# epruesse/SINA

Measured on AMD Instinct MI355X. Metric: aligned sequences/sec (whole node), 100k full-length 16S vs SILVA-NR-scale ref, higher is better.
Workload: dtype f32

## Files before the change

sina_amd/csrc/graph_build.hip:

```cpp
#include <algorithm>
#include <cstring>
#include <type_traits>

#include "common.h"
#include "ctx.h"

namespace sina_hip {
namespace {

#ifndef SINA_GRAPH_THREADS
#define SINA_GRAPH_THREADS 512
#endif
#ifndef SINA_GRAPH_MINWAVES
#define SINA_GRAPH_MINWAVES 8
#endif
constexpr int kGT = SINA_GRAPH_THREADS;
constexpr uint32_t kNoPrev = 0xFFFFu;
constexpr int kMaxFam = kFamilyMax;
#ifndef SINA_GRAPH_KTC
#define SINA_GRAPH_KTC 128
#endif
#ifndef SINA_GRAPH_TNW
#define SINA_GRAPH_TNW 512
#endif
constexpr int kTC = SINA_GRAPH_KTC;
constexpr int kTNW = SINA_GRAPH_TNW;
static_assert(kTC % 64 == 0 && kTC < 255 && kTNW >= 32 && kTNW % 2 == 0, "tile geometry");
static_assert((kMaxFam * (kTC / 64) + SINA_GRAPH_THREADS / 64 - 1) / (SINA_GRAPH_THREADS / 64) <= 64, "far-entry flags of a wave fit 64 bits");

#ifdef SINA_DP_PROFILE
__device__ unsigned long long g_graph_prof[16];
#define GP_DECL unsigned long long gp_[16] = {}; unsigned long long gt_ = __builtin_amdgcn_s_memtime();
#define GP(i) { const unsigned long long t_ = __builtin_amdgcn_s_memtime(); gp_[i] += t_ - gt_; gt_ = t_; }
#define GP_FLUSH if (threadIdx.x == 0) { for (int i_ = 0; i_ < 16; i_++) atomicAdd(&g_graph_prof[i_], gp_[i_]); }
#else
#define GP_DECL
#define GP(i)
#define GP_FLUSH
#endif

struct GraphArgs {
    const uint32_t *ref_ab;
    const uint64_t *ref_off;
    const uint32_t *fam_ids;
    const uint64_t *fam_off;
    const uint64_t *pred_off;
    const float *wtab;
    uint4 *rec;
    uint32_t *node_pos;
    uint32_t *succ_min;
    uint32_t *far_mark;
    uint32_t *pred;
    uint2 *pred4;
    uint32_t *sizes;
    uint16_t *chain_rows;
    uint32_t width, ncap;
    uint32_t tile_bytes;
    uint32_t bitmap_off;
    uint32_t member_off;
    uint32_t member_cap;
    uint32_t fam_cap;
    int W;
    int want_smin;
    uint2 *reach;
    float kappa64;
};

struct Member {
    uint64_t beg;
    uint32_t len;
    uint32_t cur, curn;
    uint32_t carry, carryn;
    uint32_t id;
};
static_assert(sizeof(Member) == 32, "LDS layout");
constexpr uint32_t kOCpos = 0;
constexpr uint32_t kONbase = kOCpos + 4 * kTC;
constexpr uint32_t kOPres = kONbase + 4 * (kTC + 2);
constexpr uint32_t kOWA = kOPres + 4 * kTC;
constexpr uint32_t kOWC = kOWA + 4 * kTNW;
constexpr uint32_t kOWD = kOWC + 4 * kTNW;
constexpr uint32_t kOWB = (kOWD + 4 * kTNW + 7) & ~7u;
constexpr uint32_t kOLi = kOWB + 8 * kTNW;
constexpr uint32_t kONn = kOLi + 32 * kTC;
constexpr uint32_t kONfar = kONn + kTC;
constexpr uint32_t kOMask = kONfar + kTNW;
constexpr uint32_t kONcol = kOMask + kTNW;
constexpr uint32_t kOE = (kONcol + kTNW + 15) & ~15u;
constexpr int kELower0Bit = 14;
constexpr uint32_t kODot16 = kTC + 1;

template <typename In, typename Out>
__device__ uint32_t block_exscan(const In *in, Out *out, uint32_t n, uint32_t *tmp) {
    const uint32_t tid = threadIdx.x;
    const uint32_t chunk = (n + kGT - 1) / kGT;
    const uint32_t b = min(n, tid * chunk), e = min(n, b + chunk);
    uint32_t s = 0;
    for (uint32_t i = b; i < e; i++) s += (uint32_t)in[i];
    uint32_t x = s;
    const int lane = tid & 63, wave = tid >> 6;
#pragma unroll
    for (int off = 1; off < 64; off <<= 1) {
        const uint32_t y = __shfl_up(x, off);
        if (lane >= off) x += y;
    }
    if (lane == 63) tmp[wave] = x;
    __syncthreads();
    uint32_t base = 0, total = 0;
    for (int w = 0; w < kGT / 64; w++) {
        if (w < wave) base += tmp[w];
        total += tmp[w];
    }
    uint32_t run = base + x - s;
    __syncthreads();
    for (uint32_t i = b; i < e; i++) {
        const uint32_t v = (uint32_t)in[i];
        out[i] = (Out)run;
        run += v;
    }
    __syncthreads();
    return total;
}

template <typename Get, typename Out>
__device__ uint32_t block_exscan_f(uint32_t n, Get get, Out *out, uint32_t *tmp) {
    const uint32_t tid = threadIdx.x;
    const uint32_t chunk = (n + kGT - 1) / kGT;
    const uint32_t b = min(n, tid * chunk), e = min(n, b + chunk);
    uint32_t s = 0;
    for (uint32_t i = b; i < e; i++) s += get(i);
    uint32_t x = s;
    const int lane = tid & 63, wave = tid >> 6;
#pragma unroll
    for (int off = 1; off < 64; off <<= 1) {
        const uint32_t y = __shfl_up(x, off);
        if (lane >= off) x += y;
    }
    if (lane == 63) tmp[wave] = x;
    __syncthreads();
    uint32_t base = 0, total = 0;
    for (int w = 0; w < kGT / 64; w++) {
        if (w < wave) base += tmp[w];
        total += tmp[w];
    }
    uint32_t run = base + x - s;
    __syncthreads();
    for (uint32_t i = b; i < e; i++) {
        const uint32_t v = get(i);
        out[i] = (Out)run;
        run += v;
    }
    __syncthreads();
    return total;
}

__device__ uint32_t block_incscan(uint32_t *v, uint32_t n, uint32_t *tmp) {
    const uint32_t tid = threadIdx.x;
    const uint32_t chunk = (n + kGT - 1) / kGT;
    const uint32_t b = min(n, tid * chunk), e = min(n, b + chunk);
    uint32_t s = 0;
    for (uint32_t i = b; i < e; i++) s += v[i];
    uint32_t x = s;
    const int lane = tid & 63, wave = tid >> 6;
#pragma unroll
    for (int off = 1; off < 64; off <<= 1) {
        const uint32_t y = __shfl_up(x, off);
        if (lane >= off) x += y;
    }
    if (lane == 63) tmp[wave] = x;
    __syncthreads();
    uint32_t base = 0, total = 0;
    for (int w = 0; w < kGT / 64; w++) {
        if (w < wave) base += tmp[w];
        total += tmp[w];
    }
    uint32_t run = base + x - s;
    for (uint32_t i = b; i < e; i++) {
        run += v[i];
        v[i] = run;
    }
    __syncthreads();
    return total;
}

constexpr uint32_t kCdSpilled = 1u << 16, kCdNone = 1u << 17, kCdSink = 1u << 30, kCdFence = 1u << 31;
__device__ __forceinline__ uint32_t row_of_code(uint32_t c) {
    return (c & kCdNone) ? kRowNone : (c & kCdSpilled) ? (kRowSpilled | (c & 0xFFFFu)) : (c & 0xFFFFu);
}

template <int K, typename Get, typename Put>
__device__ __forceinline__ uint32_t slot_walk(uint32_t b, uint32_t e, int W, Get get, Put put) {
    uint32_t fa[K];
#pragma unroll
    for (int x = 0; x < K; x++) fa[x] = (x < W) ? 0u : 0xFFFFFFFFu;
    uint32_t nsp = 0;
    for (uint32_t m = b; m < e; m++) {
        const uint32_t cd = get(m);
        const uint32_t l = cd & 0xFFFFu;
        uint32_t c = kCdNone;
        if (!(cd & kCdSink) && l != m + 1) {
            const bool may_slot = !(cd & kCdFence) && l < e;
            uint32_t slot = K;
#pragma unroll
            for (int x = K - 1; x >= 0; x--) slot = (may_slot && fa[x] <= m) ? (uint32_t)x : slot;
#pragma unroll
            for (int x = 0; x < K; x++) fa[x] = (slot == (uint32_t)x) ? l : fa[x];
            c = slot < (uint32_t)K ? slot : (kCdSpilled | nsp++);
        }
        put(m, cd, c);
    }
    return nsp;
}

__device__ __attribute__((noinline)) void fill_tile(const uint32_t *__restrict__ ref_ab, uint32_t bitmap_off, uint32_t member_off,
                                                    uint32_t nwords, uint32_t n_tasks, uint32_t c0, uint32_t tc) {
    extern __shared__ __attribute__((aligned(16))) unsigned char smem[];
    uint32_t *cposT = reinterpret_cast<uint32_t *>(smem + kOCpos);
    uint32_t *presT = reinterpret_cast<uint32_t *>(smem + kOPres);
    uint16_t *eE = reinterpret_cast<uint16_t *>(smem + kOE);
    const uint32_t *bitmap = reinterpret_cast<const uint32_t *>(smem + bitmap_off);
    const uint16_t *wrank = reinterpret_cast<const uint16_t *>(bitmap + nwords);
    Member *mb = reinterpret_cast<Member *>(smem + member_off);
    constexpr uint32_t kEAbsent = 0x00FFu, kEFirst = 1u << 13;
    constexpr uint32_t kCH = kTC / 64, kNW = kGT / 64;
    const uint32_t wave = (uint32_t)__builtin_amdgcn_readfirstlane((int)(threadIdx.x >> 6));
    const uint32_t lane = threadIdx.x & 63u;
    auto rank = [&](uint32_t pos) -> uint32_t {
        return (uint32_t)wrank[pos >> 5] + __popc(bitmap[pos >> 5] & ((1u << (pos & 31)) - 1u));
    };
        for (uint32_t t4 = wave; t4 < n_tasks; t4 += 8 * kNW) {
            uint32_t abv[8];
#pragma unroll
            for (int u = 0; u < 8; u++) {
                const uint32_t task = t4 + (uint32_t)u * kNW;
                abv[u] = 0xFFFFFFFFu;
                if (task < n_tasks) {
                    const uint32_t j = task / kCH;
                    const uint32_t cur = (uint32_t)__builtin_amdgcn_readfirstlane((int)mb[j].cur);
                    const uint32_t len = (uint32_t)__builtin_amdgcn_readfirstlane((int)mb[j].len);
                    const uint64_t beg = mb[j].beg;
                    const uint64_t begs = ((uint64_t)(uint32_t)__builtin_amdgcn_readfirstlane((int)(uint32_t)(beg >> 32)) << 32) |
                                          (uint32_t)__builtin_amdgcn_readfirstlane((int)(uint32_t)beg);
                    const uint32_t i = cur + (task % kCH) * 64u + lane;
                    if (i < len) abv[u] = ref_ab[begs + i];
                }
            }
#pragma unroll
            for (int u = 0; u < 8; u++) {
                const uint32_t task = t4 + (uint32_t)u * kNW;
                if (task >= n_tasks) continue;
                const uint32_t j = task / kCH, slot0 = (task % kCH) * 64u, slot = slot0 + lane;
                const uint32_t cur = (uint32_t)__builtin_amdgcn_readfirstlane((int)mb[j].cur);
                uint32_t ev = kEAbsent;
                if (abv[u] != 0xFFFFFFFFu) {
                    const uint32_t ab = abv[u];
                    const uint32_t pos = ab & 0xFFFFFFu;
                    const uint32_t c = rank(pos) - c0;
                    if (c < tc) {
                        const uint32_t m = (ab >> 24) & 0x1Fu;
                        ev = c | (m << 8) | (cur + slot == 0 ? kEFirst : 0u);
                        atomicOr(&presT[c], 1u << m);
                        cposT[c] = pos;
                    }
                }
                eE[j * (uint32_t)kTC + slot] = (uint16_t)ev;
                const uint32_t n_in = (uint32_t)__popcll(__builtin_amdgcn_ballot_w64(ev != kEAbsent));
                if (n_in && lane == 0) atomicMax(&mb[j].curn, cur + slot0 + n_in);
            }
        }
}

__device__ __forceinline__ uint32_t node_of_entry(uint32_t ev) {
    extern __shared__ __attribute__((aligned(16))) unsigned char smem[];
    const uint32_t *nbaseT = reinterpret_cast<const uint32_t *>(smem + kONbase);
    const uint32_t *presT = reinterpret_cast<const uint32_t *>(smem + kOPres);
    const uint8_t *liOf = smem + kOLi;
    const uint32_t c = ev & 0xFFu, m = (ev >> 8) & 31u;
    const uint32_t b = nbaseT[c];
    return b + liOf[b + __popc(presT[c] & ((1u << m) - 1u))];
}
__device__ __attribute__((noinline)) void merge_dot16(uint32_t n_tasks) {
    extern __shared__ __attribute__((aligned(16))) unsigned char smem[];
    const uint32_t *presT = reinterpret_cast<const uint32_t *>(smem + kOPres);
    uint16_t *eE = reinterpret_cast<uint16_t *>(smem + kOE);
    for (uint32_t e = threadIdx.x; e < n_tasks * 64u; e += kGT) {
        const uint32_t ev = eE[e];
        const uint32_t c = ev & 0xFFu;
        if (c != 0xFFu && ((ev >> 8) & 31u) == 16u && !(presT[c] & 0x10000u)) eE[e] = (uint16_t)((ev & ~(31u << 8)) | (1u << kELower0Bit));
    }
}
__device__ __attribute__((noinline)) void fix_dot16(uint32_t n_tasks, uint32_t ca, uint32_t cb, uint32_t w0) {
    extern __shared__ __attribute__((aligned(16))) unsigned char smem[];
    const uint32_t *nbaseT = reinterpret_cast<const uint32_t *>(smem + kONbase);
    const uint32_t *wC = reinterpret_cast<const uint32_t *>(smem + kOWC);
    const uint16_t *eE = reinterpret_cast<const uint16_t *>(smem + kOE);
    uint8_t *maskN = smem + kOMask;
    for (uint32_t e = threadIdx.x; e < n_tasks * 64u; e += kGT) {
        const uint32_t ev = eE[e];
        const uint32_t c = ev & 0xFFu;
        if (c >= ca && c < cb && (ev >> kELower0Bit) && wC[nbaseT[c] - w0] == e / (uint32_t)kTC) maskN[node_of_entry(ev) - w0] = 16;
    }
}
__global__ void __launch_bounds__(kGT) __attribute__((amdgpu_waves_per_eu(SINA_GRAPH_MINWAVES, SINA_GRAPH_MINWAVES))) family_graph_kernel(GraphArgs a) {
    extern __shared__ __attribute__((aligned(16))) unsigned char smem[];
    __shared__ uint32_t s_tmp[kGT / 64 + 8];
    const uint32_t q = blockIdx.x, tid = threadIdx.x;
    const uint32_t nwords = (a.width + 31) / 32;
    const uint64_t f0 = a.fam_off[q];
    const uint32_t F = (uint32_t)(a.fam_off[q + 1] - f0);
    uint32_t *cposT = reinterpret_cast<uint32_t *>(smem + kOCpos);
    uint32_t *nbaseT = reinterpret_cast<uint32_t *>(smem + kONbase);
    uint32_t *presT = reinterpret_cast<uint32_t *>(smem + kOPres);
    uint32_t *wA = reinterpret_cast<uint32_t *>(smem + kOWA);
    uint32_t *wC = reinterpret_cast<uint32_t *>(smem + kOWC);
    uint32_t *wD = reinterpret_cast<uint32_t *>(smem + kOWD);
    unsigned long long *wB = reinterpret_cast<unsigned long long *>(smem + kOWB);
    uint8_t *liOf = smem + kOLi;
    uint8_t *nn = smem + kONn;
    uint8_t *nfarN = smem + kONfar;
    uint8_t *maskN = smem + kOMask;
    uint8_t *ncolN = smem + kONcol;
    uint16_t *eE = reinterpret_cast<uint16_t *>(smem + kOE);
    uint32_t *bitmap = reinterpret_cast<uint32_t *>(smem + a.bitmap_off);
    uint16_t *wrank = reinterpret_cast<uint16_t *>(bitmap + nwords);
    Member *mb = reinterpret_cast<Member *>(smem + a.member_off);
    constexpr uint32_t kEFirst = 1u << 13;
    constexpr uint32_t kCH = kTC / 64, kNW = kGT / 64;
    const uint32_t wave = (uint32_t)__builtin_amdgcn_readfirstlane((int)(threadIdx.x >> 6));
    const uint32_t lane = threadIdx.x & 63u;
    const uint32_t n_tasks = F * kCH;

    uint32_t *sz = a.sizes + kBuiltWords * (size_t)q;
    for (uint32_t j = tid; j < F; j += kGT) {
        const uint32_t id = a.fam_ids[f0 + j];
        mb[j].id = id;
        mb[j].beg = a.ref_off[id];
        mb[j].len = (uint32_t)(a.ref_off[id + 1] - a.ref_off[id]);
        mb[j].cur = mb[j].curn = 0;
        mb[j].carry = mb[j].carryn = kNoPrev;
    }
    for (uint32_t i = tid; i < nwords; i += kGT) bitmap[i] = 0;
    if (tid == 0) nbaseT[kODot16] = 0;
    __syncthreads();
    GP_DECL

    for (uint32_t j0 = 0; j0 < F; j0 += 8) {
        uint32_t maxlen = 0;
#pragma unroll
        for (int u = 0; u < 8; u++) maxlen = max(maxlen, j0 + u < F ? mb[j0 + u].len : 0u);
        for (uint32_t i = tid; i < maxlen; i += kGT) {
            uint32_t ab[8];
#pragma unroll
            for (int u = 0; u < 8; u++)
                ab[u] = (j0 + u < F && i < mb[j0 + u].len) ? a.ref_ab[mb[j0 + u].beg + i] : 0xFFFFFFFFu;
#pragma unroll
            for (int u = 0; u < 8; u++)
                if (ab[u] != 0xFFFFFFFFu) {
                    const uint32_t pos = ab[u] & 0xFFFFFFu;
                    atomicOr(&bitmap[pos >> 5], 1u << (pos & 31));
                }
        }
    }
    __syncthreads();
    GP(0)
    {
        const uint32_t chunk = (nwords + kGT - 1) / kGT;
        const uint32_t b = min(nwords, tid * chunk), e = min(nwords, b + chunk);
        uint32_t s = 0;
        for (uint32_t i = b; i < e; i++) s += __popc(bitmap[i]);
        uint32_t x = s;
        const int lane = tid & 63, wave = tid >> 6;
#pragma unroll
        for (int off = 1; off < 64; off <<= 1) {
            const uint32_t y = __shfl_up(x, off);
            if (lane >= off) x += y;
        }
        if (lane == 63) s_tmp[wave] = x;
        __syncthreads();
        uint32_t base = 0, total = 0;
        for (int w = 0; w < kGT / 64; w++) {
            if (w < wave) base += s_tmp[w];
            total += s_tmp[w];
        }
        uint32_t run = base + x - s;
        for (uint32_t i = b; i < e; i++) {
            wrank[i] = (uint16_t)run;
            run += __popc(bitmap[i]);
        }
        if (tid == 0) s_tmp[kGT / 64] = total;
    }
    __syncthreads();
    const uint32_t NC = s_tmp[kGT / 64];
    if (NC > 65535u) {
        if (tid == 0) {
            sz[kBuiltN] = NC;
            sz[kBuiltEdges] = sz[kBuiltSpill] = 0;
            sz[kBuiltStatus] = kBuiltNodeCap;
        }
        return;
    }
    auto rank = [&](uint32_t pos) -> uint32_t {
        return (uint32_t)wrank[pos >> 5] + __popc(bitmap[pos >> 5] & ((1u << (pos & 31)) - 1u));
    };
    uint4 *rec = a.rec + (size_t)q * a.ncap;
    uint32_t *node_pos = a.node_pos + (size_t)q * a.ncap;
    uint32_t *smin = a.succ_min + (size_t)q * a.ncap;
    uint32_t *last = a.far_mark + (size_t)q * a.ncap;
    uint32_t *pred = a.pred + a.pred_off[q];
    uint16_t *chain_rows = a.chain_rows + (size_t)q * a.ncap;
    const float *wt = a.wtab + (size_t)F * (kMaxFam + 1);
    uint32_t N = 0, E = 0;
    GP(1)

    for (uint32_t c0 = 0; c0 < NC; c0 += kTC) {
        const uint32_t tc = min((uint32_t)kTC, NC - c0);
        for (uint32_t i = tid; i < (uint32_t)kTC; i += kGT) presT[i] = 0;
        __syncthreads();
        GP(2)
        fill_tile(a.ref_ab, a.bitmap_off, a.member_off, nwords, n_tasks, c0, tc);
        __syncthreads();
        for (uint32_t c = tid; c < tc; c += kGT) {
            uint32_t p = presT[c];
            if ((p & 0x10001u) == 0x10001u) {
                p &= ~0x10000u;
                presT[c] = p;
                nbaseT[kODot16] = 1u;
            }
            nn[c] = (uint8_t)__popc(p);
        }
        __syncthreads();
        if (nbaseT[kODot16]) {
            merge_dot16(n_tasks);
            __syncthreads();
        }
        GP(3)
        const uint32_t tn = block_exscan(nn, nbaseT, tc, s_tmp);
        if (tid == 0) nbaseT[tc] = tn;
        for (uint32_t ln = tid; ln < tn; ln += kGT)
            if (N + ln < a.ncap) {
                last[N + ln] = 0;
                if (a.want_smin) smin[N + ln] = 0xFFFFFFFFu;
            }
        __syncthreads();
        GP(5)
        uint32_t te = 0;
        for (uint32_t ca = 0; ca < tc;) {
            const uint32_t w0 = nbaseT[ca];
            uint32_t cb = tc;
            if (tn - w0 > (uint32_t)kTNW) {
                uint32_t lo = ca + 1, hi = tc;
                while (lo < hi) {
                    const uint32_t mid = (lo + hi + 1) / 2;
                    if (nbaseT[mid] - w0 <= (uint32_t)kTNW) lo = mid;
                    else hi = mid - 1;
                }
                cb = lo;
            }
            const uint32_t wn = nbaseT[cb] - w0;
            for (uint32_t i = tid; i < wn; i += kGT) {
                wA[i] = 0;
                wB[i] = 0;
                wC[i] = 0xFFFFFFFFu;
                nfarN[i] = 0;
            }
            __syncthreads();
            for (uint32_t task = wave; task < n_tasks; task += kNW) {
                const uint32_t j = task / kCH, slot = (task % kCH) * 64u + lane;
                const uint32_t ev = eE[j * (uint32_t)kTC + slot];
                const uint32_t c = ev & 0xFFu;
                if (c >= ca && c < cb) {
                    const uint32_t m = (ev >> 8) & 31u;
                    atomicMin(&wC[nbaseT[c] + __popc(presT[c] & ((1u << m) - 1u)) - w0], j);
                }
            }
            __syncthreads();
            for (uint32_t c = ca + tid; c < cb; c += kGT) {
                const uint32_t base = nbaseT[c], k = nn[c];
                uint32_t pp = presT[c];
                for (uint32_t x = 0; x < k; x++) {
                    const uint32_t mj = wC[base - w0 + x];
                    uint32_t r = 0;
                    for (uint32_t y = 0; y < k; y++) r += (wC[base - w0 + y] < mj) ? 1u : 0u;
                    liOf[base + x] = (uint8_t)r;
                    maskN[base - w0 + r] = (uint8_t)(__ffs(pp) - 1);
                    ncolN[base - w0 + r] = (uint8_t)c;
                    pp &= pp - 1u;
                }
            }
            __syncthreads();
            if (nbaseT[kODot16]) {
                fix_dot16(n_tasks, ca, cb, w0);
                __syncthreads();
            }
            GP(4)
            auto node_of = [&](uint32_t ev) -> uint32_t { return node_of_entry(ev); };
            unsigned long long farbits = 0;
            {
                uint32_t it = 0;
                for (uint32_t task = wave; task < n_tasks; task += kNW, it++) {
                    const uint32_t j = task / kCH, slot = (task % kCH) * 64u + lane;
                    const uint32_t ev = eE[j * (uint32_t)kTC + slot];
                    const uint32_t c = ev & 0xFFu;
                    const bool mine = c >= ca && c < cb;
                    const uint32_t ln = mine ? node_of(ev) : 0u;
                    uint32_t lnp = __shfl_up(ln, 1);
                    const bool left_mine = __shfl_up(mine ? 1 : 0, 1) != 0;
                    if (!mine) continue;
                    const uint32_t node = N + ln;
                    const bool first = (ev & kEFirst) != 0;
                    atomicAdd(&wA[ln - w0], first ? 1u : 0x10001u);
                    if (mb[j].cur + slot + 1 == mb[j].curn) mb[j].carryn = node;
                    if (j == 0 && mb[0].cur + slot < a.ncap) chain_rows[mb[0].cur + slot] = (uint16_t)node;
                    if (!first) {
                        if (slot && (lane == 0 || !left_mine)) lnp = node_of(eE[j * (uint32_t)kTC + slot - 1]);
                        const uint32_t pn = slot ? N + lnp : mb[j].carry;
                        const uint32_t d = node - pn;
                        if (d <= 64u) atomicOr(&wB[ln - w0], 1ull << (d - 1u));
                        else farbits |= 1ull << it;
                    }
                }
            }
            for (uint32_t i = tid; i < wn; i += kGT) wC[i] = 0xFFFFFFFFu;
            __syncthreads();
            GP(6)
            const uint32_t te_w = block_exscan_f(wn, [&](uint32_t i) { return wA[i] >> 16; }, wD, s_tmp);
            while (__syncthreads_or(farbits != 0 ? 1 : 0)) {
                uint32_t it = 0;
                for (uint32_t task = wave; task < n_tasks; task += kNW, it++) {
                    if (!((farbits >> it) & 1ull)) continue;
                    const uint32_t j = task / kCH, slot = (task % kCH) * 64u + lane;
                    const uint32_t ln = node_of(eE[j * (uint32_t)kTC + slot]);
                    const uint32_t pn = slot ? N + node_of(eE[j * (uint32_t)kTC + slot - 1]) : mb[j].carry;
                    atomicMin(&wC[ln - w0], pn);
                }
                __syncthreads();
                it = 0;
                for (uint32_t task = wave; task < n_tasks; task += kNW, it++) {
                    if (!((farbits >> it) & 1ull)) continue;
                    const uint32_t j = task / kCH, slot = (task % kCH) * 64u + lane;
                    const uint32_t ln = node_of(eE[j * (uint32_t)kTC + slot]);
                    const uint32_t pn = slot ? N + node_of(eE[j * (uint32_t)kTC + slot - 1]) : mb[j].carry;
                    if (wC[ln - w0] == pn) farbits &= ~(1ull << it);
                }
                __syncthreads();
                for (uint32_t i = tid; i < wn; i += kGT) {
                    const uint32_t v = wC[i];
                    if (v == 0xFFFFFFFFu) continue;
                    const uint32_t node = N + w0 + i;
                    if (node < a.ncap) {
                        pred[E + te + wD[i] + nfarN[i]] = v;
                        if (a.want_smin) atomicMin(&smin[v], cposT[ncolN[i]]);
                        atomicMax(&last[v], node);
                    }
                    nfarN[i]++;
                    wC[i] = 0xFFFFFFFFu;
                }
            }
            for (uint32_t i = tid; i < wn; i += kGT) {
                const uint32_t node = N + w0 + i;
                if (node >= a.ncap) continue;
                const uint32_t seg = E + te + wD[i];
                const uint32_t pos = cposT[ncolN[i]];
                uint32_t np = nfarN[i];
                unsigned long long bits = wB[i];
                while (bits) {
                    const uint32_t hi = 63u - (uint32_t)__clzll((long long)bits);
                    bits ^= 1ull << hi;
                    const uint32_t pa = node - (hi + 1u);
                    pred[seg + np] = pa;
                    np++;
                    if (a.want_smin) atomicMin(&smin[pa], pos);
                    atomicMax(&last[pa], node);
                }
                uint4 r;
                r.x = seg;
                r.y = __float_as_uint(wt[wA[i] & 0xFFFFu]);
                r.z = (np & 0xFFu) | ((uint32_t)maskN[i] << 8);
                r.w = kRowNone;
                rec[node] = r;
                node_pos[node] = pos;
            }
            te += te_w;
            ca = cb;
            __syncthreads();
        }
        for (uint32_t j = tid; j < F; j += kGT) {
            mb[j].cur = mb[j].curn;
            mb[j].carry = mb[j].carryn;
        }
        N += tn;
        E += te;
        __syncthreads();
        GP(7)
    }
    if (N > a.ncap || N > 65535u) {
        if (tid == 0) {
            sz[kBuiltN] = N;
            sz[kBuiltEdges] = sz[kBuiltSpill] = 0;
            sz[kBuiltStatus] = kBuiltNodeCap;
        }
        return;
    }
    GP(8)
    const uint32_t seg_len = dp_slot_segment(N);
    const uint32_t n_seg = (N + seg_len - 1) / seg_len;
    uint32_t *codeL = reinterpret_cast<uint32_t *>(smem);
    const bool in_lds = (size_t)N * 4 <= a.tile_bytes;
    const bool beside = a.reach != nullptr && (size_t)N * 8 <= a.tile_bytes;
    uint32_t *cwL = codeL + N;
    constexpr int kSFirstSink = kGT / 64 + 1, kSGmin = kGT / 64 + 2, kSSpill = kGT / 64 + 3;
    if (tid == 0) {
        s_tmp[kSFirstSink] = 0xFFFFFFFFu;
        s_tmp[kSGmin] = 0xFFFFFFFFu;
    }
    __syncthreads();
    for (uint32_t i = tid; i < N; i += kGT) {
        const uint32_t l = last[i];
        uint32_t cd = l;
        if (l == 0) {
            cd |= kCdSink;
            atomicMin(&s_tmp[kSFirstSink], i);
            if (a.want_smin) smin[i] = 1000000u;
        }
        if (l > i && l - i > (uint32_t)kFarLds) cd |= kCdFence;
        if (in_lds) codeL[i] = cd;
        else if (cd & (kCdSink | kCdFence)) rec[i].z |= ((cd & kCdSink) ? kRecSink : 0u) | ((cd & kCdFence) ? kRecFence : 0u);
    }
    auto column_maxima = [&](uint32_t *cw, uint32_t first, uint32_t step) {
        for (uint32_t i = first; i < N; i += step) {
            const uint32_t pos = node_pos[i];
            if (i > 0 && node_pos[i - 1] == pos) continue;
            uint32_t mx = 0;
            for (uint32_t j = i; j < N && node_pos[j] == pos; j++) {
                mx = max(mx, prune_gain_units(__uint_as_float(rec[j].y), a.kappa64));
                cw[j] = 0;
            }
            cw[i] = mx;
            atomicMin(&s_tmp[kSGmin], mx);
        }
    };
    __syncthreads();
    GP(9)
    if (wave == 0) {
        uint32_t nsp = 0;
        if (tid < n_seg) {
            const uint32_t b = tid * seg_len, e = min(N, b + seg_len);
            auto walk = [&](auto kslots) {
                constexpr int K = decltype(kslots)::value;
                if (in_lds)
                    return slot_walk<K>(b, e, a.W, [&](uint32_t m) { return codeL[m]; },
                                        [&](uint32_t m, uint32_t cd, uint32_t c) { codeL[m] = (cd & (kCdSink | kCdFence)) | c; });
                return slot_walk<K>(b, e, a.W,
                                    [&](uint32_t m) {
                                        const uint32_t z = rec[m].z;
                                        return last[m] | ((z & kRecSink) ? kCdSink : 0u) | ((z & kRecFence) ? kCdFence : 0u);
                                    },
                                    [&](uint32_t m, uint32_t, uint32_t c) { rec[m].w = row_of_code(c); });
            };
            nsp = (a.W <= 4) ? walk(std::integral_constant<int, 4>()) : walk(std::integral_constant<int, 8>());
        }
        uint32_t x = nsp;
#pragma unroll
        for (int off = 1; off < 16; off <<= 1) {
            const uint32_t y = __shfl_up(x, off);
            if (lane >= (uint32_t)off) x += y;
        }
        if (tid < n_seg) mb[tid].id = x - nsp;
        if (tid == 15) s_tmp[kSSpill] = x;
    } else if (beside) {
        column_maxima(cwL, tid - 64u, (uint32_t)kGT - 64u);
    }
    __syncthreads();
    const uint32_t tot = s_tmp[kSSpill];
    if (tid == 0) {
        sz[kBuiltN] = N;
        sz[kBuiltEdges] = E;
        sz[kBuiltSpill] = tot;
        sz[kBuiltStatus] = (tot > kMaxSpillRows) ? kBuiltSpillCap : 0u;
        sz[kBuiltFirstSink] = s_tmp[kSFirstSink];
        sz[kBuiltChainLen] = mb[0].len;
        if (beside) sz[kBuiltGmin] = s_tmp[kSGmin];
    }
    uint2 *pred4 = a.pred4 + (size_t)q * a.ncap;
    uint2 *rg = a.reach + (size_t)q * a.ncap;
    if (in_lds) {
        for (uint32_t i = tid; i < N; i += kGT) {
            const uint32_t c = codeL[i];
            if (c & kCdSpilled) codeL[i] = c + mb[i / seg_len].id;
        }
        uint32_t total = 0;
        if (beside) total = block_incscan(cwL, N, s_tmp);
        else __syncthreads();
        GP(10)
        for (uint32_t i = tid; i < N; i += kGT) {
            const uint4 r = rec[i];
            const uint32_t cd = codeL[i];
            const uint32_t np = r.z & 0xFFu;
            uint32_t first_far = 0;
            uint32_t dist = np ? 0u : kRecDistFar;
            uint32_t p4[4] = {0u, 0u, 0u, 0u};
            for (uint32_t x = 0; x < np; x++) {
                const uint32_t pa = pred[r.x + x];
                const uint32_t pc = codeL[pa];
                const bool sp = (pc & kCdSpilled) != 0;
                if (sp && first_far == 0) first_far = x + 1;
                dist = max(dist, i - pa);
                pred[r.x + x] = pa | ((pc & 0x7FFFu) << 16) | (sp ? kPredSpilled : 0u);
                if (x == 0) p4[0] = pa;
                else if (x == 1) p4[1] = pa;
                else if (x == 2) p4[2] = pa;
                else if (x == 3) p4[3] = pa;
            }
            uint4 o;
            o.x = r.x;
            o.y = r.y;
            o.z = r.z | ((cd & kCdSink) ? kRecSink : 0u) | ((cd & kCdFence) ? kRecFence : 0u) | (first_far << 24) |
                  (min(dist, kRecDistFar) << kRecDistShift);
            o.w = row_of_code(cd);
            rec[i] = o;
            pred4[i] = pred4_pack(p4[0], p4[1], p4[2], p4[3]);
            if (beside) rg[i] = uint2{total - cwL[i], last[i] | ((NC - 1u - rank(node_pos[i])) << 16)};
        }
        GP(11)
        if (a.reach != nullptr && !beside) {
            __syncthreads();
            column_maxima(codeL, tid, (uint32_t)kGT);
            __syncthreads();
            if (tid == 0) sz[kBuiltGmin] = s_tmp[kSGmin];
            total = block_incscan(codeL, N, s_tmp);
            for (uint32_t i = tid; i < N; i += kGT)
                rg[i] = uint2{total - codeL[i], last[i] | ((NC - 1u - rank(node_pos[i])) << 16)};
        }
        GP(12)
    } else {
        for (uint32_t i = tid; i < N; i += kGT) {
            const uint32_t w = rec[i].w;
            if (w != kRowNone && (w & kRowSpilled)) rec[i].w = w + mb[i / seg_len].id;
        }
        __syncthreads();
        GP(10)
        for (uint32_t i = tid; i < N; i += kGT) {
            const uint4 r = rec[i];
            const uint32_t np = r.z & 0xFFu;
            uint32_t first_far = 0;
            uint32_t dist = np ? 0u : kRecDistFar;
            uint32_t p4[4] = {0u, 0u, 0u, 0u};
            for (uint32_t x = 0; x < np; x++) {
                const uint32_t pa = pred[r.x + x];
                uint32_t pw = rec[pa].w;
                if (pw == kRowNone) pw = 0;
                const bool sp = (pw & kRowSpilled) != 0;
                if (sp && first_far == 0) first_far = x + 1;
                dist = max(dist, i - pa);
                pred[r.x + x] = pa | ((pw & 0x7FFFu) << 16) | (sp ? kPredSpilled : 0u);
                if (x == 0) p4[0] = pa;
                else if (x == 1) p4[1] = pa;
                else if (x == 2) p4[2] = pa;
                else if (x == 3) p4[3] = pa;
            }
            rec[i].z = r.z | (first_far << 24) | (min(dist, kRecDistFar) << kRecDistShift);
            pred4[i] = pred4_pack(p4[0], p4[1], p4[2], p4[3]);
        }
        GP(11)
        if (a.reach != nullptr) {
            uint32_t *cw = a.want_smin ? last : smin;
            column_maxima(cw, tid, (uint32_t)kGT);
            __syncthreads();
            if (tid == 0) sz[kBuiltGmin] = s_tmp[kSGmin];
            const uint32_t total = block_exscan(cw, cw, N, s_tmp);
            for (uint32_t i = tid; i < N; i += kGT) {
                const uint32_t pos = node_pos[i];
                if (i > 0 && node_pos[i - 1] == pos) continue;
                const uint32_t right = (i + 1 < N) ? total - cw[i + 1] : 0u;
                const uint32_t cols_right = NC - 1u - rank(pos);
                for (uint32_t j = i; j < N && node_pos[j] == pos; j++) rg[j] = uint2{right, (a.want_smin ? 0u : last[j]) | (cols_right << 16)};
            }
        }
        GP(12)
    }
    GP_FLUSH
}

size_t graph_bitmap_off(uint32_t max_family) { return ((size_t)kOE + 2 * (size_t)max_family * kTC + 15) & ~(size_t)15; }
size_t graph_lds_bytes(uint32_t width, uint32_t max_family) {
    const size_t nwords = (width + 31) / 32;
    return graph_bitmap_off(max_family) + ((6 * nwords + 15) & ~(size_t)15);
}
size_t graph_member_cap(uint32_t max_family) { return std::max<size_t>(16, (max_family + 1) & ~(size_t)1); }
size_t graph_lds_total(uint32_t width, uint32_t max_family) {
    return graph_lds_bytes(width, max_family) + sizeof(Member) * graph_member_cap(max_family);
}

}
}

using namespace sina_hip;

namespace {

int build_family_graphs(sina_hip_ctx *c, const uint32_t *fam_ids, const uint64_t *fam_off, uint32_t q0,
                        uint32_t bq, float fs_weight, int W, BuiltGraphs *bg, bool want_smin, float kappa64, bool for_dp) {
    hipStream_t s = c->stream;
    if (ensure_ref_off_host(c)) return 1;
    std::vector<uint64_t> foff(bq + 1), elems(bq, 0);
    uint32_t max_f = 1;
    bg->pred_off.assign(bq, 0);
    for (uint32_t q = 0; q <= bq; q++) foff[q] = fam_off[q0 + q] - fam_off[q0];
    for (uint32_t q = 0; q < bq; q++) {
        max_f = std::max<uint32_t>(max_f, (uint32_t)(foff[q + 1] - foff[q]));
        for (uint64_t x = fam_off[q0 + q]; x < fam_off[q0 + q + 1]; x++) {
            const uint32_t id = fam_ids[x];
            if (id >= c->st->n_refs) SH_FAIL("align_families: reference id out of range");
            elems[q] += c->st->ref_off_host[id + 1] - c->st->ref_off_host[id];
        }
        if (for_dp && elems[q] == 0) SH_FAIL("align_families: a family without a single base");
    }
    if (!(c->wtab_fs_weight == fs_weight) || !c->g_wtab.p) {
        std::vector<float> wt((size_t)(kMaxFam + 1) * (kMaxFam + 1), 0.f);
        const float weight = fs_weight;
        for (unsigned F = 1; F <= (unsigned)kMaxFam; F++)
            for (unsigned cnt = 0; cnt <= F; cnt++)
                wt[(size_t)F * (kMaxFam + 1) + cnt] =
                    (float)(1.0 / (double)(weight + 1) + (double)(weight * ((float)cnt / (float)F)));
        if (c->g_wtab.reserve(wt.size() * 4)) return 1;
        SH_CHECK(hipMemcpyAsync(c->g_wtab.p, wt.data(), wt.size() * 4, hipMemcpyHostToDevice, s));
        SH_CHECK(hipStreamSynchronize(s));
        c->wtab_fs_weight = fs_weight;
    }
    uint32_t ncap = std::min<uint32_t>(65535, 12288);
    for (int attempt = 0;; attempt++) {
        uint64_t pred_total = 0;
        for (uint32_t q = 0; q < bq; q++) {
            bg->pred_off[q] = pred_total;
            pred_total += elems[q] + 8;
        }
        const size_t glds_tables = graph_lds_bytes(c->st->width, max_f);
        const size_t glds = graph_lds_total(c->st->width, max_f);
        if (glds > 160 * 1024) SH_FAIL_LIMIT("align_families: family too wide for the device DAG build");
        if (c->g_fam_ids.reserve(4 * std::max<uint64_t>(foff[bq], 1)) || c->g_fam_off.reserve(8 * ((uint64_t)bq + 1)) ||
            c->g_tmp1.reserve(8 * (uint64_t)bq) ||
            c->rec.reserve(sizeof(uint4) * (uint64_t)bq * ncap) || c->node_pos.reserve(4 * (uint64_t)bq * ncap) ||
            c->succ_minpos.reserve(4 * (uint64_t)bq * ncap) || c->g_tmp3.reserve(4 * (uint64_t)bq * ncap) ||
            c->pred.reserve(4 * pred_total) || c->pred4.reserve(sizeof(uint2) * (uint64_t)bq * ncap) || c->g_sizes.reserve(4 * kBuiltWords * (uint64_t)bq) ||
            c->scout.reserve(2 * (uint64_t)bq * ncap) ||
            (kappa64 > 0.f && c->rgain.reserve(8 * (uint64_t)bq * ncap)))
            return 1;
        if (upload(c, 1, c->g_fam_ids.p, fam_ids + fam_off[q0], 4 * foff[bq], s) ||
            upload(c, 2, c->g_fam_off.p, foff.data(), 8 * ((uint64_t)bq + 1), s) ||
            upload(c, 3, c->g_tmp1.p, bg->pred_off.data(), 8 * (uint64_t)bq, s))
            return 1;
        GraphArgs ga;
        ga.ref_ab = c->st->ref_ab.as<uint32_t>();
        ga.ref_off = c->st->ref_off.as<uint64_t>();
        ga.fam_ids = c->g_fam_ids.as<uint32_t>();
        ga.fam_off = c->g_fam_off.as<uint64_t>();
        ga.pred_off = c->g_tmp1.as<uint64_t>();
        ga.wtab = c->g_wtab.as<float>();
        ga.rec = c->rec.as<uint4>();
        ga.node_pos = c->node_pos.as<uint32_t>();
        ga.succ_min = c->succ_minpos.as<uint32_t>();
        ga.far_mark = c->g_tmp3.as<uint32_t>();
        ga.pred = c->pred.as<uint32_t>();
        ga.pred4 = c->pred4.as<uint2>();
        ga.sizes = c->g_sizes.as<uint32_t>();
        ga.chain_rows = c->scout.as<uint16_t>();
        ga.width = c->st->width;
        ga.ncap = ncap;
        ga.bitmap_off = (uint32_t)graph_bitmap_off(max_f);
        ga.tile_bytes = ga.bitmap_off;
        ga.member_off = (uint32_t)glds_tables;
        ga.member_cap = (uint32_t)graph_member_cap(max_f);
        ga.fam_cap = max_f;
        ga.W = W;
        ga.want_smin = want_smin ? 1 : 0;
        ga.reach = kappa64 > 0.f ? c->rgain.as<uint2>() : nullptr;
        ga.kappa64 = kappa64;
        if (allow_full_lds(reinterpret_cast<const void *>(family_graph_kernel))) return 1;
        bg->sizes.resize(kBuiltWords * (size_t)bq);
        {
            heavy_launch hl(c, s, kHeavyGraph);
            SH_CHECK(hipEventRecord(c->ev[6], hl.stream()));
            hipLaunchKernelGGL(family_graph_kernel, dim3(bq), dim3(kGT), glds, hl.stream(), ga);
            SH_CHECK(hipGetLastError());
            SH_CHECK(hipEventRecord(c->ev[7], hl.stream()));
            if (hl.done()) return 1;
        }
        if (download(c, 4, c->g_sizes.p, 4 * kBuiltWords * (uint64_t)bq, s)) return 1;
        SH_CHECK(wait_stream(c, s));
        memcpy(bg->sizes.data(), c->h_stage[4].p, 4 * kBuiltWords * (uint64_t)bq);
        float gms = 0;
        SH_CHECK(hipEventElapsedTime(&gms, c->ev[6], c->ev[7]));
        {
            uint64_t bytes = 0;
            for (uint32_t q = 0; q < bq; q++)
                bytes += 4 * elems[q] + (uint64_t)bg->sizes[kBuiltWords * q + kBuiltN] * (16 + 4 + 8 + (kappa64 > 0.f ? 8 : 0)) +
                         4 * (uint64_t)bg->sizes[kBuiltWords * q + kBuiltEdges];
            std::lock_guard<std::mutex> slk(c->st->stats_mu);
            c->st->stats.graph_ms += gms;
            c->st->stats.graph_bytes += bytes;
            c->st->stats.graph_launches++;
        }
        uint32_t need_n = 0;
        for (uint32_t q = 0; q < bq; q++) {
            const uint32_t status = bg->sizes[kBuiltWords * q + kBuiltStatus];
            if (status == kBuiltNodeCap) need_n = std::max(need_n, bg->sizes[kBuiltWords * q + kBuiltN]);
            if (status == kBuiltSpillCap) SH_FAIL_LIMIT("align_families: too many spill rows for one query");
        }
        if (!need_n) break;
        if (attempt >= 3 || need_n > 65535u) SH_FAIL_LIMIT("align_families: family DAG exceeds device limits");
        ncap = std::min<uint32_t>(65535, need_n + need_n / 8 + 16);
    }
    bg->ncap = ncap;
    return 0;
}

int build_graphs_for_launch(sina_hip_ctx *c, const uint32_t *fam_ids, const uint64_t *fam_off, uint32_t q0, uint32_t n,
                            const sina_hip_align_params *p, int W, const PrunePlan &pp, BuiltGraphs *bg) {
    return build_family_graphs(c, fam_ids, fam_off, q0, n, p->fs_weight, W, bg, p->insertion == SINA_INSERTION_FORBID,
                               pp.on ? pp.kappa64 : 0.f, true);
}

}

extern "C" {

int sina_hip_align_families(sina_hip_ctx *c, const uint32_t *fam_ids, const uint64_t *fam_off, uint32_t nq,
                            const uint8_t *qmask, const uint64_t *qoff, const sina_hip_align_params *p,
                            sina_hip_align_out *out, uint32_t *out_pos) {
    return align_family_batches(c, FamilyCall{"align_families", build_graphs_for_launch, false, fam_ids, fam_off, nq, qmask, qoff, p, out, out_pos});
}

int sina_hip_align_families_wsets(sina_hip_ctx *c, const uint32_t *fam_ids, const uint64_t *fam_off, uint32_t nq,
                                  const uint8_t *qmask, const uint64_t *qoff, const sina_hip_align_params *p,
                                  const uint32_t *weight_set, uint32_t n_sets, sina_hip_align_out *out, uint32_t *out_pos) {
    if (p && !weighted_scheme(p)) SH_FAIL("align_families_wsets: weight sets need positional weights (p->weights, p->n_weights)");
    return align_family_batches(c, FamilyCall{"align_families_wsets", build_graphs_for_launch, false, fam_ids, fam_off, nq, qmask, qoff, p,
                                             out, out_pos, weight_set, n_sets});
}

#ifdef SINA_DP_PROFILE
int sina_hip_debug_graph_profile(unsigned long long *out16, int reset) {
    SH_CHECK(hipMemcpyFromSymbol(out16, HIP_SYMBOL(g_graph_prof), sizeof(unsigned long long) * 16));
    if (reset) {
        unsigned long long z[16] = {};
        SH_CHECK(hipMemcpyToSymbol(HIP_SYMBOL(g_graph_prof), z, sizeof z));
    }
    return 0;
}
#endif

int sina_hip_debug_family_graph(sina_hip_ctx *c, const uint32_t *fam_ids, uint32_t F, float fs_weight,
                                uint32_t ring_depth, uint32_t *n_nodes, uint32_t *n_edges, uint32_t *pos,
                                uint8_t *mask, float *weight, uint32_t *pred_off, uint32_t *pred,
                                uint32_t *succ_minpos, uint8_t *sink, uint32_t *spill_idx, uint32_t cap_nodes,
                                uint32_t cap_edges) {
    if (!c || !fam_ids || !n_nodes || !n_edges) SH_FAIL("debug_family_graph: null argument");
    std::lock_guard<std::mutex> lk(c->mu);
    if (!c->st->have_refs) SH_FAIL("debug_family_graph: upload references first");
    if (F == 0 || F > (uint32_t)kMaxFam) SH_FAIL("debug_family_graph: family size must be in 1..128");
    SH_CHECK(hipSetDevice(c->device));
    const uint64_t foff[2] = {0, F};
    BuiltGraphs bg;
    if (build_family_graphs(c, fam_ids, foff, 0, 1, fs_weight, (int)ring_depth, &bg, true, fs_weight >= 0.f ? 64.0f * 1.0001f * 2.0f : 0.f, false)) return 1;
    const uint32_t N = bg.sizes[kBuiltN];
    std::vector<uint4> rec(N);
    std::vector<uint32_t> pr(bg.sizes[kBuiltEdges] + 8);
    SH_CHECK(hipMemcpy(rec.data(), c->rec.p, sizeof(uint4) * N, hipMemcpyDeviceToHost));
    SH_CHECK(hipMemcpy(pr.data(), c->pred.p, 4 * pr.size(), hipMemcpyDeviceToHost));
    uint32_t E = 0;
    for (uint32_t m = 0; m < N; m++) E += rec[m].z & 0xffu;
    *n_nodes = N;
    *n_edges = E;
    if (N > cap_nodes || E > cap_edges) SH_FAIL("debug_family_graph: output buffers too small");
    SH_CHECK(hipMemcpy(pos, c->node_pos.p, 4 * N, hipMemcpyDeviceToHost));
    SH_CHECK(hipMemcpy(succ_minpos, c->succ_minpos.p, 4 * N, hipMemcpyDeviceToHost));
    uint32_t e = 0;
    for (uint32_t m = 0; m < N; m++) {
        mask[m] = (uint8_t)((rec[m].z >> 8) & 0xffu);
        memcpy(&weight[m], &rec[m].y, 4);
        sink[m] = (rec[m].z & kRecSink) ? 1 : 0;
        spill_idx[m] = rec[m].w;
        pred_off[m] = e;
        for (uint32_t x = 0; x < (rec[m].z & 0xffu); x++) pred[e++] = pr[rec[m].x + x] & 0xffffu;
    }
    pred_off[N] = e;
    return 0;
}

int sina_hip_debug_family_graph_words(sina_hip_ctx *c, const uint32_t *fam_ids, uint32_t F, float fs_weight,
                                      uint32_t ring_depth, uint32_t *n_nodes, uint32_t *n_edges, uint32_t *rec_z,
                                      uint32_t *rec_w, uint32_t *pred_entries, uint32_t *size_words, uint32_t cap_nodes,
                                      uint32_t cap_edges) {
    if (!c || !fam_ids || !n_nodes || !n_edges || !rec_z || !rec_w || !pred_entries || !size_words)
        SH_FAIL("debug_family_graph_words: null argument");
    std::lock_guard<std::mutex> lk(c->mu);
    if (!c->st->have_refs) SH_FAIL("debug_family_graph_words: upload references first");
    if (F == 0 || F > (uint32_t)kMaxFam) SH_FAIL("debug_family_graph_words: family size must be in 1..128");
    SH_CHECK(hipSetDevice(c->device));
    const uint64_t foff[2] = {0, F};
    BuiltGraphs bg;
    if (build_family_graphs(c, fam_ids, foff, 0, 1, fs_weight, (int)ring_depth, &bg, true, fs_weight >= 0.f ? 64.0f * 1.0001f * 2.0f : 0.f, false)) return 1;
    const uint32_t N = bg.sizes[kBuiltN];
    std::vector<uint4> rec(N);
    std::vector<uint32_t> pr(bg.sizes[kBuiltEdges] + 8);
    if (N) SH_CHECK(hipMemcpy(rec.data(), c->rec.p, sizeof(uint4) * N, hipMemcpyDeviceToHost));
    SH_CHECK(hipMemcpy(pr.data(), c->pred.p, 4 * pr.size(), hipMemcpyDeviceToHost));
    uint32_t E = 0;
    for (uint32_t m = 0; m < N; m++) E += rec[m].z & 0xffu;
    *n_nodes = N;
    *n_edges = E;
    if (N > cap_nodes || E > cap_edges) SH_FAIL("debug_family_graph_words: output buffers too small");
    uint32_t e = 0;
    for (uint32_t m = 0; m < N; m++) {
        rec_z[m] = rec[m].z;
        rec_w[m] = rec[m].w;
        for (uint32_t x = 0; x < (rec[m].z & 0xffu); x++) pred_entries[e++] = pr[rec[m].x + x];
    }
    memcpy(size_words, bg.sizes.data(), 4 * kBuiltWords);
    return 0;
}

}
```

Baseline: 310,500.

## Cut block barriers in graph-build tile loop via single-pass column scan

Replaces the per-tile presence fixup, separate exclusive scan and reset pass with one thread-per-column scan that also flags dot merges. It folds the far-edge vote into the edge exclusive scan, so the first syncthreads_or is dropped, and moves presT clearing and member cursor updates into the last window iteration. The aim is fewer __syncthreads per tile in the graph-build kernel. The catch is subtle ordering: barriers removed inside block_exscan and presT zeroing relies on later barriers, which risks races if the assumptions fail.

```diff
diff --git a/sina_amd/csrc/graph_build.hip b/sina_amd/csrc/graph_build.hip
--- a/sina_amd/csrc/graph_build.hip
+++ b/sina_amd/csrc/graph_build.hip
@@ -112,7 +112,6 @@
         total += tmp[w];
     }
     uint32_t run = base + x - s;
-    __syncthreads();
     for (uint32_t i = b; i < e; i++) {
         const uint32_t v = (uint32_t)in[i];
         out[i] = (Out)run;
@@ -123,7 +122,7 @@
 }
 
 template <typename Get, typename Out>
-__device__ uint32_t block_exscan_f(uint32_t n, Get get, Out *out, uint32_t *tmp) {
+__device__ uint32_t block_exscan_f(uint32_t n, Get get, Out *out, uint32_t *tmp, bool vote, bool *any) {
     const uint32_t tid = threadIdx.x;
     const uint32_t chunk = (n + kGT - 1) / kGT;
     const uint32_t b = min(n, tid * chunk), e = min(n, b + chunk);
@@ -136,15 +135,18 @@
         const uint32_t y = __shfl_up(x, off);
         if (lane >= off) x += y;
     }
-    if (lane == 63) tmp[wave] = x;
-    __syncthreads();
-    uint32_t base = 0, total = 0;
+    const uint32_t wave_vote = __builtin_amdgcn_ballot_w64(vote) != 0 ? 0x80000000u : 0u;
+    if (lane == 63) tmp[wave] = x | wave_vote;
+    __syncthreads();
+    uint32_t base = 0, total = 0, votes = 0;
     for (int w = 0; w < kGT / 64; w++) {
-        if (w < wave) base += tmp[w];
-        total += tmp[w];
-    }
+        const uint32_t t = tmp[w];
+        if (w < wave) base += t & 0x7FFFFFFFu;
+        total += t & 0x7FFFFFFFu;
+        votes |= t;
+    }
+    *any = (votes & 0x80000000u) != 0;
     uint32_t run = base + x - s;
-    __syncthreads();
     for (uint32_t i = b; i < e; i++) {
         const uint32_t v = get(i);
         out[i] = (Out)run;
@@ -179,6 +181,54 @@
         run += v[i];
         v[i] = run;
     }
+    __syncthreads();
+    return total;
+}
+
+static_assert(kTC <= kGT, "a thread per tile column");
+__device__ __forceinline__ uint32_t tile_column_scan(uint32_t tc, uint32_t *tmp) {
+    extern __shared__ __attribute__((aligned(16))) unsigned char smem[];
+    uint32_t *nbaseT = reinterpret_cast<uint32_t *>(smem + kONbase);
+    uint32_t *presT = reinterpret_cast<uint32_t *>(smem + kOPres);
+    uint8_t *nn = smem + kONn;
+    constexpr int kCW = kTC / 64;
+    const uint32_t tid = threadIdx.x;
+    const int lane = tid & 63, wave = tid >> 6;
+    uint32_t p = 0;
+    bool merged = false;
+    if (tid < tc) {
+        p = presT[tid];
+        if ((p & 0x10001u) == 0x10001u) {
+            p &= ~0x10000u;
+            merged = true;
+        }
+    }
+    const uint32_t s = __popc(p);
+    uint32_t x = s;
+    if (wave < kCW) {
+#pragma unroll
+        for (int off = 1; off < 64; off <<= 1) {
+            const uint32_t y = __shfl_up(x, off);
+            if (lane >= off) x += y;
+        }
+        if (lane == 63) tmp[wave] = x;
+    }
+    __syncthreads();
+    uint32_t base = 0, total = 0;
+#pragma unroll
+    for (int w = 0; w < kCW; w++) {
+        if (w < wave) base += tmp[w];
+        total += tmp[w];
+    }
+    if (tid < tc) {
+        nn[tid] = (uint8_t)s;
+        (presT + tid)[((int)kONbase - (int)kOPres) / 4] = base + x - s;
+        if (merged) {
+            presT[tid] = p;
+            nbaseT[kODot16] = 1u;
+        }
+    }
+    if (tid == 0) nbaseT[tc] = total;
     __syncthreads();
     return total;
 }
@@ -340,6 +390,7 @@
         mb[j].carry = mb[j].carryn = kNoPrev;
     }
     for (uint32_t i = tid; i < nwords; i += kGT) bitmap[i] = 0;
+    for (uint32_t i = tid; i < (uint32_t)kTC; i += kGT) presT[i] = 0;
     if (tid == 0) nbaseT[kODot16] = 0;
     __syncthreads();
     GP_DECL
@@ -414,35 +465,10 @@
 
     for (uint32_t c0 = 0; c0 < NC; c0 += kTC) {
         const uint32_t tc = min((uint32_t)kTC, NC - c0);
-        for (uint32_t i = tid; i < (uint32_t)kTC; i += kGT) presT[i] = 0;
-        __syncthreads();
-        GP(2)
         fill_tile(a.ref_ab, a.bitmap_off, a.member_off, nwords, n_tasks, c0, tc);
         __syncthreads();
-        for (uint32_t c = tid; c < tc; c += kGT) {
-            uint32_t p = presT[c];
-            if ((p & 0x10001u) == 0x10001u) {
-                p &= ~0x10000u;
-                presT[c] = p;
-                nbaseT[kODot16] = 1u;
-            }
-            nn[c] = (uint8_t)__popc(p);
-        }
-        __syncthreads();
-        if (nbaseT[kODot16]) {
-            merge_dot16(n_tasks);
-            __syncthreads();
-        }
         GP(3)
-        const uint32_t tn = block_exscan(nn, nbaseT, tc, s_tmp);
-        if (tid == 0) nbaseT[tc] = tn;
-        for (uint32_t ln = tid; ln < tn; ln += kGT)
-            if (N + ln < a.ncap) {
-                last[N + ln] = 0;
-                if (a.want_smin) smin[N + ln] = 0xFFFFFFFFu;
-            }
-        __syncthreads();
-        GP(5)
+        const uint32_t tn = tile_column_scan(tc, s_tmp);
         uint32_t te = 0;
         for (uint32_t ca = 0; ca < tc;) {
             const uint32_t w0 = nbaseT[ca];
@@ -463,7 +489,16 @@
                 wC[i] = 0xFFFFFFFFu;
                 nfarN[i] = 0;
             }
+            if (ca == 0) {
+                for (uint32_t ln = tid; ln < tn; ln += kGT)
+                    if (N + ln < a.ncap) {
+                        last[N + ln] = 0;
+                        if (a.want_smin) smin[N + ln] = 0xFFFFFFFFu;
+                    }
+                if (nbaseT[kODot16]) merge_dot16(n_tasks);
+            }
             __syncthreads();
+            GP(5)
             for (uint32_t task = wave; task < n_tasks; task += kNW) {
                 const uint32_t j = task / kCH, slot = (task % kCH) * 64u + lane;
                 const uint32_t ev = eE[j * (uint32_t)kTC + slot];
@@ -523,8 +558,9 @@
             for (uint32_t i = tid; i < wn; i += kGT) wC[i] = 0xFFFFFFFFu;
             __syncthreads();
             GP(6)
-            const uint32_t te_w = block_exscan_f(wn, [&](uint32_t i) { return wA[i] >> 16; }, wD, s_tmp);
-            while (__syncthreads_or(farbits != 0 ? 1 : 0)) {
+            bool far;
+            const uint32_t te_w = block_exscan_f(wn, [&](uint32_t i) { return wA[i] >> 16; }, wD, s_tmp, farbits != 0, &far);
+            for (; far; far = __syncthreads_or(farbits != 0 ? 1 : 0) != 0) {
                 uint32_t it = 0;
                 for (uint32_t task = wave; task < n_tasks; task += kNW, it++) {
                     if (!((farbits >> it) & 1ull)) continue;
@@ -580,17 +616,19 @@
                 rec[node] = r;
                 node_pos[node] = pos;
             }
+            if (cb == tc) {
+                for (uint32_t j = tid; j < F; j += kGT) {
+                    mb[j].cur = mb[j].curn;
+                    mb[j].carry = mb[j].carryn;
+                }
+                for (uint32_t i = tid; i < (uint32_t)kTC; i += kGT) presT[i] = 0;
+            }
             te += te_w;
             ca = cb;
             __syncthreads();
         }
-        for (uint32_t j = tid; j < F; j += kGT) {
-            mb[j].cur = mb[j].curn;
-            mb[j].carry = mb[j].carryn;
-        }
         N += tn;
         E += te;
-        __syncthreads();
         GP(7)
     }
     if (N > a.ncap || N > 65535u) {
```

Result: no change. 310,000 (median of 3 runs) (-0.1%).
